# mmp/pbrt-v3

Measured on NVIDIA H100. Metric: Msamples/sec, higher is better.
Workload: dtype f32

## Files before the change

include/pb2.h:

```cpp
#ifndef PB2_H
#define PB2_H

#include <stddef.h>
#include <stdint.h>

#ifdef __cplusplus
extern "C" {
#endif

#define PB2_ABI_VERSION 10

typedef enum pb2_status {
    PB2_OK = 0,
    PB2_ERR_NO_DEVICE = 1,
    PB2_ERR_CUDA = 2,
    PB2_ERR_INVALID = 3,
    PB2_ERR_UNSUPPORTED = 4,
    PB2_ERR_NCCL = 5
} pb2_status;


typedef struct pb2_bvh_node {
    float bmin[3];
    float bmax[3];
    int32_t offset;
    uint16_t n_prims;
    uint8_t axis;
    uint8_t pad;
} pb2_bvh_node;

enum { PB2_PRIM_TRIANGLE = 0, PB2_PRIM_SPHERE = 1, PB2_PRIM_INSTANCE = 2 };
enum { PB2_MAT_NONE = 0, PB2_MAT_MATTE = 1, PB2_MAT_PLASTIC = 2, PB2_MAT_MIRROR = 3, PB2_MAT_GLASS = 4, PB2_MAT_SUBSTRATE = 5, PB2_MAT_METAL = 6,
       PB2_MAT_UBER = 7 };
enum { PB2_LIGHTDIST_UNIFORM = 0, PB2_LIGHTDIST_POWER = 1, PB2_LIGHTDIST_SPATIAL = 2 };
enum { PB2_FILTER_BOX = 0, PB2_FILTER_GAUSSIAN = 1, PB2_FILTER_MITCHELL = 2, PB2_FILTER_SINC = 3, PB2_FILTER_TRIANGLE = 4 };

typedef struct pb2_mesh {
    int32_t first_tri, n_tris;
    int32_t first_vertex, n_vertices;
    int32_t has_n, has_uv, has_s;
    int32_t reverse_orientation;
    int32_t transform_swaps_handedness;
    int32_t alpha_tex, shadow_alpha_tex;
    int32_t pad;
} pb2_mesh;

enum { PB2_WRAP_REPEAT = 0, PB2_WRAP_BLACK = 1, PB2_WRAP_CLAMP = 2 };
typedef struct pb2_texture {
    int32_t channels;
    int32_t width, height;
    int32_t wrap;
    int32_t do_trilinear;
    float max_anisotropy;
    float su, sv, du, dv;
    int32_t kind;
    int32_t pad;
    const float *texels;
    int32_t child[3];
    float value[3];
} pb2_texture;
enum { PB2_TEXKIND_IMAGE = 0, PB2_TEXKIND_CONSTANT = 1, PB2_TEXKIND_SCALE = 2, PB2_TEXKIND_MIX = 3, PB2_TEXKIND_CHECKERBOARD = 4,
       PB2_TEXKIND_UV = 5 };

enum { PB2_TEX_KD = 0, PB2_TEX_KS = 1, PB2_TEX_KR = 2, PB2_TEX_KT = 3, PB2_TEX_OPACITY = 4, PB2_TEX_SIGMA = 5, PB2_TEX_ROUGHNESS = 6,
       PB2_TEX_UROUGHNESS = 7, PB2_TEX_VROUGHNESS = 8, PB2_TEX_ETA = 9, PB2_TEX_METAL_ETA = 10, PB2_TEX_METAL_K = 11,
       PB2_TEX_BUMP = 12, PB2_TEX_SLOTS = 13 };

typedef struct pb2_sphere {
    float object_to_world[16];
    float world_to_object[16];
    float radius, z_min, z_max, theta_min, theta_max, phi_max;
    int32_t reverse_orientation;
    int32_t transform_swaps_handedness;
} pb2_sphere;

typedef struct pb2_material {
    int32_t type;
    float kd[3];
    float sigma;
    float ks[3];
    float roughness;
    int32_t remap_roughness;
    int32_t pad[2];
    float kr[3];
    float kt[3];
    float eta;
    float uroughness, vroughness;
    float opacity[3];
    float metal_eta[3];
    float metal_k[3];
    int32_t pad3[2];
    int32_t tex[16];
} pb2_material;

enum { PB2_LIGHT_AREA = 0, PB2_LIGHT_POINT = 1, PB2_LIGHT_SPOT = 2, PB2_LIGHT_DISTANT = 3, PB2_LIGHT_INFINITE = 4 };
typedef struct pb2_light {
    int32_t prim;
    float L[3];
    int32_t two_sided;
    float area;
    int32_t type;
    int32_t pad;
} pb2_light;

typedef struct pb2_delta_light {
    float p[3];
    float total_width_deg;
    float falloff_start_deg;
    float world_radius;
    float world_to_light[9];
    float pad;
    float light_to_world[9];
    int32_t env_tex;
    float pad2[2];
} pb2_delta_light;

typedef struct pb2_bvh {
    int64_t node_offset, n_nodes;
    int64_t prim_offset, n_prims;
} pb2_bvh;

typedef struct pb2_instance {
    float instance_to_world[16];
    float world_to_instance[16];
    int32_t bvh;
    int32_t lone_prim;
    int32_t pad[2];
} pb2_instance;

typedef struct pb2_scene_desc {
    int64_t n_vertices;
    const float *P;
    const float *N;
    const float *UV;
    const float *S;
    int64_t n_tris;
    const int32_t *tri_index;
    const int32_t *tri_mesh;
    int32_t n_meshes;
    const pb2_mesh *meshes;
    int32_t n_spheres;
    const pb2_sphere *spheres;

    int64_t n_prims;
    const uint8_t *prim_type;
    const int32_t *prim_index;
    const int32_t *prim_material;
    const int32_t *prim_light;

    int64_t n_nodes;
    const pb2_bvh_node *nodes;
    const int32_t *bvh_prims;

    int32_t n_materials;
    const pb2_material *materials;
    int32_t n_lights;
    const pb2_light *lights;

    int32_t light_strategy;
    int32_t spatial_max_voxels;

    int32_t n_instances;
    int32_t n_bvhs;
    const pb2_instance *instances;
    const pb2_bvh *bvhs;
    int64_t n_bvh_prims;
    const pb2_delta_light *delta_lights;
    int32_t n_textures;
    int32_t pad_textures;
    const pb2_texture *textures;
} pb2_scene_desc;

typedef struct pb2_camera {
    float camera_to_world[16];
    float world_to_camera[16];
    float screen_window[4];
    float fov;
    float lens_radius, focal_distance;
    float shutter_open, shutter_close;
    float raster_to_camera[16];
    float dx_camera[3], dy_camera[3];
} pb2_camera;

typedef struct pb2_film_desc {
    int32_t full_resolution[2];
    int32_t cropped_pixel_bounds[4];
    float filter_radius[2];
    float max_sample_luminance;
    float scale;
    int32_t filter_type;
    float filter_param[2];
    int32_t pad;
} pb2_film_desc;

typedef struct pb2_path_params {
    int32_t samples_per_pixel;
    int32_t sample_at_pixel_center;
    int32_t max_depth;
    float rr_threshold;
    int32_t pixel_bounds[4];
    int32_t tile_rank, tile_count;
    int32_t flags;
    int32_t sampler;
} pb2_path_params;

enum { PB2_SAMPLER_HALTON = 0, PB2_SAMPLER_SOBOL = 1 };

#define PB2_FLAG_COUNT_TRAVERSAL 1
#define PB2_FLAG_LINEAR_NODES 2
#define PB2_FLAG_WIDE4 4
#define PB2_FLAG_PLAIN_TRACE 8
#define PB2_FLAG_SMALL_STACK 16
#define PB2_FLAG_LD128 32
#define PB2_FLAG_LEAF_TMA 64
#define PB2_FLAG_POOL 128
#define PB2_FLAG_CHAIN 256

typedef struct pb2_ray {
    float o[3];
    float d[3];
    float t_max;
} pb2_ray;

typedef struct pb2_hit {
    int32_t prim;
    float t;
    float b[3];
    float p[3];
    float p_error[3];
    float n[3];
    float ns[3];
    float dpdu[3];
    float uv[2];
} pb2_hit;

typedef struct pb2_stats {
    uint64_t camera_rays;
    uint64_t regular_rays;
    uint64_t shadow_rays;
    uint64_t node_visits;
    uint64_t prim_tests;
    uint64_t kernel_launches;
    double render_ms;
    double h2d_ms, d2h_ms;
    double trace_ms;
} pb2_stats;

typedef struct pb2_scene pb2_scene;


int pb2_abi_version(void);
const char *pb2_last_error(void);

int pb2_init(int device_id);
int pb2_init_devices(int n_devices, const int *device_ids);
int pb2_device_count(void);
int pb2_shutdown(void);

#define PB2_DIST_ID_BYTES 128
int pb2_dist_unique_id(void *id);
int pb2_dist_init(int rank, int world, const void *id);
int pb2_dist_info(int *rank, int *world);
int pb2_dist_shutdown(void);

int pb2_work_items(const pb2_film_desc *film, const pb2_path_params *params, int64_t first, int64_t n, int32_t *out,
                   int64_t *n_items);

int pb2_host_alloc(size_t bytes, void **out);
int pb2_host_free(void *p);

int pb2_scene_create(const pb2_scene_desc *desc, pb2_scene **out);
int pb2_scene_destroy(pb2_scene *scene);
int pb2_shade_class(const pb2_scene_desc *desc, int32_t *out);

int pb2_intersect(pb2_scene *scene, const pb2_ray *rays, int64_t n, pb2_hit *hits);
int pb2_intersect_p(pb2_scene *scene, const pb2_ray *rays, int64_t n, uint8_t *occluded);

int pb2_render_path(pb2_scene *scene, const pb2_camera *camera, const pb2_film_desc *film,
                    const pb2_path_params *params, float *film_rgbw, pb2_stats *stats);

int pb2_render_path_device(pb2_scene *scene, const pb2_camera *camera, const pb2_film_desc *film,
                           const pb2_path_params *params, float *film_rgbw_device, int clear,
                           void *stream, pb2_stats *stats);

typedef struct pb2_wf_hit {
    int32_t found;
    int32_t leaf;
    int32_t prim;
    float t;
    float b[3];
    int32_t listed;
} pb2_wf_hit;
int pb2_trace_wavefront(pb2_scene *scene, const pb2_ray *rays, const uint8_t *any_hit, int64_t n, int32_t flags,
                        pb2_wf_hit *out);

int pb2_li_samples(pb2_scene *scene, const pb2_camera *camera, const pb2_film_desc *film,
                   const pb2_path_params *params, const int32_t *pixel_xy, const int64_t *sample_num,
                   int64_t n, float *out_rgb, float *out_pfilm);

int pb2_halton_samples(const pb2_film_desc *film, const pb2_path_params *params,
                       const int32_t *pixel_xy, const int64_t *sample_num, const int32_t *dim,
                       int64_t n, float *out);

int pb2_sobol_samples_host(const pb2_film_desc *film, const pb2_path_params *params, const int32_t *pixel_xy,
                           const int64_t *sample_num, const int32_t *dim, int64_t n, float *out, uint64_t *tables);

int pb2_light_distribution(pb2_scene *scene, const float *points_xyz, int64_t n, float *out);

int pb2_texture_pyramid(const pb2_texture *texture, int32_t level, int32_t *n_levels, int32_t *w, int32_t *h, float *out);

int pb2_texture_eval_host(const pb2_texture *textures, int32_t n_textures, int32_t id, int64_t n, const float *uv, const float *duv,
                          float *out);

int pb2_bsdf_eval_host(const pb2_material *material, int64_t n, const float *in, float *out);

int pb2_camera_differentials_host(const pb2_camera *camera, const pb2_film_desc *film, const pb2_path_params *params, int64_t n,
                                  const float *in, float *out);
int pb2_uv_differentials_host(int64_t n, const float *in, float *out);

int pb2_env_distribution(const pb2_texture *texture, int32_t *nu, int32_t *nv, float *out);

int pb2_texture_lookup(const pb2_texture *texture, int64_t n, const float *st, const float *dst, float *out);

typedef struct pb2_build_node {
    float bmin[3], bmax[3];
    int32_t child[2];
    int32_t split_axis;
    int32_t first_prim_offset;
    int32_t n_primitives;
} pb2_build_node;
int pb2_hlbvh_treelets(const float *prim_bounds, int64_t n, int32_t max_prims_in_node, pb2_build_node *pool,
                       int32_t *ordered_prims, int32_t *treelet_roots, int32_t *n_treelets, double *device_ms);

int pb2_hlbvh_build(const float *prim_bounds, int64_t n, int32_t max_prims_in_node, pb2_bvh_node *nodes, int64_t *n_nodes,
                    int32_t *ordered_prims, double *device_ms);

#ifdef __cplusplus
}
#endif
#endif
```

pbrt_v3_b200/csrc/pb2_cuda.cu:

```cuda
#include <cuda_runtime.h>
#include <cub/device/device_radix_sort.cuh>
#include <dlfcn.h>
#include <nccl.h>

#include <algorithm>
#include <mutex>
#include <chrono>
#include <cstddef>
#include <cstdio>
#include <cstdlib>
#include <cstring>
#include <string>
#include <thread>
#include <vector>

#include "device/pb2_path.cuh"
#include "device/pb2_wide4.cuh"
#include "host/core.h"
#include "pb2.h"

using namespace pb2;

static thread_local std::string g_lastError;
static int setError(int code, const std::string &msg) {
// ... 486 lines not shown
    int s = r >> 8, m = r & 255;
    int x = rp.sbx0 + tx * 16 + compact1by1((unsigned)m);
    int y = rp.sby0 + ty * 16 + compact1by1((unsigned)m >> 1);
    *px = x;
    *py = y;
    *sample = s;
    if (x >= rp.sbx1 || y >= rp.sby1) return false;
    return x >= rp.pbx0 && x < rp.pbx1 && y >= rp.pby0 && y < rp.pby1;
}

__device__ __noinline__ void addSampleFiltered(const DRenderParams &rp, float4 *film, V2 pFilm, V3 L) {
    float dx = pFilm.x - 0.5f, dy = pFilm.y - 0.5f;
    int p0x = (int)ceilf(dx - rp.filterRadiusX), p0y = (int)ceilf(dy - rp.filterRadiusY);
    int p1x = (int)floorf(dx + rp.filterRadiusX) + 1, p1y = (int)floorf(dy + rp.filterRadiusY) + 1;
    p0x = max(p0x, rp.cx0);
    p0y = max(p0y, rp.cy0);
    p1x = min(p1x, rp.cx1);
    p1y = min(p1y, rp.cy1);
    int width = rp.cx1 - rp.cx0;
    for (int yy = p0y; yy < p1y; ++yy) {
        float fy = fabsf(((float)yy - dy) * rp.invFilterRadiusY * 16.f);
        int ify = min((int)floorf(fy), 15);
        for (int xx = p0x; xx < p1x; ++xx) {
            float fx = fabsf(((float)xx - dx) * rp.invFilterRadiusX * 16.f);
            int ifx = min((int)floorf(fx), 15);
            float w = rp.filterTable[ify * 16 + ifx];
            float4 *px = film + ((size_t)(yy - rp.cy0) * width + (xx - rp.cx0));
            atomicAdd(px, make_float4(L.x * w, L.y * w, L.z * w, w));
        }
    }
}

__device__ __forceinline__ void addSample(const DRenderParams &rp, float4 *film, V2 pFilm, V3 L) {
    float y = luminance(L);
    if (y > rp.maxSampleLuminance) L = L * (rp.maxSampleLuminance / y);
    if (rp.filterTable) {
        addSampleFiltered(rp, film, pFilm, L);
        return;
    }
    float dx = pFilm.x - 0.5f, dy = pFilm.y - 0.5f;
    int p0x = (int)ceilf(dx - rp.filterRadiusX), p0y = (int)ceilf(dy - rp.filterRadiusY);
    int p1x = (int)floorf(dx + rp.filterRadiusX) + 1, p1y = (int)floorf(dy + rp.filterRadiusY) + 1;
    p0x = max(p0x, rp.cx0);
    p0y = max(p0y, rp.cy0);
    p1x = min(p1x, rp.cx1);
    p1y = min(p1y, rp.cy1);
    int width = rp.cx1 - rp.cx0;
    for (int yy = p0y; yy < p1y; ++yy)
        for (int xx = p0x; xx < p1x; ++xx) {
            float4 *px = film + ((size_t)(yy - rp.cy0) * width + (xx - rp.cx0));
            atomicAdd(px, make_float4(L.x, L.y, L.z, 1.f));
        }
}

#include "pb2_wavefront.cuh"

__global__ void k_li_samples(DScene sc, DRenderParams rp, const int32_t *pixelXY, const int64_t *sampleNum, int64_t n,
                             float *outRGB, float *outPFilm, int *deferred) {
    int64_t i = blockIdx.x * (int64_t)blockDim.x + threadIdx.x;
    if (i >= n) return;
    int px = pixelXY[2 * i], py = pixelXY[2 * i + 1];
    DSampler smp;
    smp.index = sampleIndex<true>(rp.halton, px, py, sampleNum[i]);
    smp.dim = 0;
    V2 pFilm;
    DRay ray = generateCameraRay<true>(rp.cam, rp.halton, smp, px, py, &pFilm);
    DLane ln;
    laneStartPath(ln, ray, smp);
    while (ln.state != LS_IDLE) {
        DHit hit;
        float tMax;
        bool found = traceLane(sc, ln, &tMax, &hit, nullptr);
        DTexCtx tc;
        tc.cam = &rp.cam;
        tc.pFilm = pFilm;
        tc.diffScale = rp.diffScale;
        laneAdvance<SHADE_FULL>(sc, rp.halton, rp.path, ln, found, hit, tMax, &tc);
        if (ln.state == LS_DEFER) {
            atomicAdd(deferred, 1);
            return;
        }
    }
    V3 L = guardRadiance(ln.L);
    outRGB[3 * i] = L.x;
    outRGB[3 * i + 1] = L.y;
    outRGB[3 * i + 2] = L.z;
    if (outPFilm) {
        outPFilm[2 * i] = pFilm.x;
        outPFilm[2 * i + 1] = pFilm.y;
    }
}

__global__ void k_wf_debug_fill(WfPool pool, const pb2_ray *rays, const uint8_t *anyHit, int n) {
    int i = blockIdx.x * blockDim.x + threadIdx.x;
    if (i == 0) {
        for (int q = 0; q < WQ_COUNT; ++q) pool.counts[q] = 0;
        pool.counts[WQ_TRACE0] = (unsigned)n;
    }
    if (i >= n) return;
    WfCtx &cx = pool.ctx[i];
    cx.ln.state = (anyHit && anyHit[i]) ? LS_SHADOW : LS_PATH;
    cx.ln.ray.o = mk3(rays[i].o[0], rays[i].o[1], rays[i].o[2]);
    cx.ln.ray.d = mk3(rays[i].d[0], rays[i].d[1], rays[i].d[2]);
    cx.ln.ray.tMax = rays[i].t_max;
    cx.hit = make_float4(__int_as_float(-1), 0.f, 0.f, 0.f);
    cx.tHit = 0.f;
    cx.found = -1;
    pool.queue[WQ_TRACE0][i] = i;
}
__global__ void k_wf_debug_read(DScene sc, WfPool pool, int n, pb2_wf_hit *out) {
    int i = blockIdx.x * blockDim.x + threadIdx.x;
    if (i >= n) return;
    const WfCtx &cx = pool.ctx[i];
    pb2_wf_hit h;
    h.found = cx.found;
    h.t = cx.tHit;
    h.leaf = __float_as_int(cx.hit.x);
    h.b[0] = cx.hit.y; h.b[1] = cx.hit.z; h.b[2] = cx.hit.w;
    h.prim = (cx.found > 0 && h.leaf >= 0) ? asInt(ldg4(&sc.leafPrims[3 * (size_t)h.leaf]).w) : -1;
    h.listed = 0;
    out[i] = h;
}
__global__ void k_wf_debug_lists(WfPool pool, pb2_wf_hit *out) {
    unsigned ns = pool.counts[WQ_SHADE], nl = pool.counts[WQ_LIGHT];
    for (unsigned i = blockIdx.x * blockDim.x + threadIdx.x; i < ns + nl; i += gridDim.x * blockDim.x) {
        int c = i < ns ? pool.queue[WQ_SHADE][i] : pool.queue[WQ_LIGHT][i - ns];
        atomicAdd(&out[c].listed, i < ns ? 1 : 2);
    }
}

__global__ void k_halton_samples(DHalton h, const int32_t *pixelXY, const int64_t *sampleNum, const int32_t *dim, int64_t n,
                                 float *out) {
    int64_t i = blockIdx.x * (int64_t)blockDim.x + threadIdx.x;
    if (i >= n) return;
    const int px = pixelXY[2 * i], py = pixelXY[2 * i + 1];
    int64_t index = sampleIndex<true>(h, px, py, sampleNum[i]);
    if (h.sobol && dim[i] < 2) out[i] = sobolPixelSample(h, index, dim[i], dim[i] == 0 ? px : py);
    else out[i] = sampleDimension<true>(h, index, dim[i]);
}

__global__ void k_halton_batch(DHalton h, const int32_t *pixelXY, const int64_t *sampleNum, const int32_t *dim0, int64_t n, float *out) {
    int64_t i = blockIdx.x * (int64_t)blockDim.x + threadIdx.x;
    if (i >= n) return;
    const int64_t index = sampleIndex<true>(h, pixelXY[2 * i], pixelXY[2 * i + 1], sampleNum[i]);
    float u[kSampleBatch];
    haltonSampleBatch<true>(h, index, dim0[i], kSampleBatch, u);
#pragma unroll
    for (int k = 0; k < kSampleBatch; ++k) out[kSampleBatch * i + k] = u[k];
}

__global__ void k_light_distribution(DScene sc, const float *points, int64_t n, float *out) {
    int64_t i = blockIdx.x * (int64_t)blockDim.x + threadIdx.x;
    if (i >= n) return;
    const float *rec = lightDistLookup(sc.lightDist, mk3(points[3 * i], points[3 * i + 1], points[3 * i + 2]));
    if (!rec) return;
    int stride = 2 * sc.nLights + 1;
    for (int k = 0; k < stride; ++k) out[i * stride + k] = rec[k];
}

static DHalton haltonTablesOnly() {
    DHalton h;
    memset(&h, 0, sizeof(h));
    h.primes = cur().primes;
    h.primeSums = cur().primeSums;
    h.perms = cur().perms;
    h.dimRecs = cur().dimRecs;
    h.dimTabs = cur().dimTabs;
    h.digitTab = cur().digitTab;
    return h;
}

static void launchLightDistBuild(const pb2_scene *scene, cudaStream_t stream) {
    k_lightdist_build<<<g_numSMs * 4, 128, 0, stream>>>(scene->d, haltonTablesOnly());
    k_lightdist_done<<<1, 32, 0, stream>>>(scene->d);
}
static int lightDistOverflowed(pb2_scene *scene, cudaStream_t stream, bool *overflowed) {
    *overflowed = false;
    if (!scene->lazyLightDist) return PB2_OK;
    CUDA_TRY(cudaMemcpyAsync(scene->ldHostCounters, scene->d.lightDist.counters, 4 * sizeof(int), cudaMemcpyDeviceToHost, stream));
    CUDA_TRY(cudaStreamSynchronize(stream));
    *overflowed = scene->ldHostCounters[2] != 0;
    return PB2_OK;
}
static int lightDistOverflowError() {
    return setError(PB2_ERR_UNSUPPORTED, "the on-demand pool of spatial light distributions is exhausted (very many lights x very many voxels touched): "
                                         "raise PB2_LIGHTDIST_POOL_MB or use lightsamplestrategy \"power\" / \"uniform\"");
}

static int requireDevice() {
    if (!g_initialised) return setError(PB2_ERR_NO_DEVICE, "pb2_init() has not succeeded: no CUDA device is bound (there is no CPU fallback)");
    return PB2_OK;
}

static bool computeFilterTable(const pb2_film_desc *f, float table[256]) {
    const float rx = f->filter_radius[0], ry = f->filter_radius[1];
    const float p0 = f->filter_param[0], p1 = f->filter_param[1];
    auto eval = [&](float x, float y) -> float {
        switch (f->filter_type) {
        case PB2_FILTER_GAUSSIAN: {
            const float alpha = p0, expX = std::exp(-alpha * rx * rx), expY = std::exp(-alpha * ry * ry);
            auto g = [&](float d, float expv) { return std::max((float)0, float(std::exp(-alpha * d * d) - expv)); };
            return g(x, expX) * g(y, expY);
        }
        case PB2_FILTER_MITCHELL: {
            const float B = p0, C = p1;
            auto m1 = [&](float v) {
                v = std::abs(2 * v);
                if (v > 1)
                    return ((-B - 6 * C) * v * v * v + (6 * B + 30 * C) * v * v + (-12 * B - 48 * C) * v + (8 * B + 24 * C)) * (1.f / 6.f);
                return ((12 - 9 * B - 6 * C) * v * v * v + (-18 + 12 * B + 6 * C) * v * v + (6 - 2 * B)) * (1.f / 6.f);
            };
            const float invRx = 1 / rx, invRy = 1 / ry;
            return m1(x * invRx) * m1(y * invRy);
        }
        case PB2_FILTER_SINC: {
            const float tau = p0, Pi = 3.14159265358979323846f;
            auto sinc = [&](float v) -> float {
                v = std::abs(v);
                if (v < 1e-5) return 1;
                return std::sin(Pi * v) / (Pi * v);
            };
            auto ws = [&](float v, float radius) -> float {
                v = std::abs(v);
                if (v > radius) return 0;
                float lanczos = sinc(v / tau);
                return sinc(v) * lanczos;
            };
            return ws(x, rx) * ws(y, ry);
        }
        case PB2_FILTER_TRIANGLE:
            return std::max((float)0, rx - std::abs(x)) * std::max((float)0, ry - std::abs(y));
        default:
            return 1.f;
        }
    };
    int offset = 0;
    for (int y = 0; y < 16; ++y)
        for (int x = 0; x < 16; ++x, ++offset) table[offset] = eval((x + 0.5f) * rx / 16, (y + 0.5f) * ry / 16);
    return f->filter_type != PB2_FILTER_BOX;
}

static DRenderParams makeRenderParams(const pb2_camera *cam, const pb2_film_desc *film, const pb2_path_params *pp) {
    DRenderParams rp;
    memset(&rp, 0, sizeof(rp));
    memcpy(rp.cam.rasterToCamera.m, cam->raster_to_camera, sizeof(float) * 16);
    memcpy(rp.cam.cameraToWorld.m, cam->camera_to_world, sizeof(float) * 16);
    rp.cam.lensRadius = cam->lens_radius;
    rp.cam.focalDistance = cam->focal_distance;
    rp.cam.dxCamera = mk3(cam->dx_camera[0], cam->dx_camera[1], cam->dx_camera[2]);
    rp.cam.dyCamera = mk3(cam->dy_camera[0], cam->dy_camera[1], cam->dy_camera[2]);
    rp.diffScale = 1 / std::sqrt((float)pp->samples_per_pixel);
    rp.halton = makeHalton(film, pp);
    rp.path.maxDepth = pp->max_depth;
    rp.path.rrThreshold = pp->rr_threshold;
    SampleBounds sb = filmSampleBounds(film);
    rp.sbx0 = sb.x0; rp.sby0 = sb.y0; rp.sbx1 = sb.x1; rp.sby1 = sb.y1;
    rp.pbx0 = pp->pixel_bounds[0]; rp.pby0 = pp->pixel_bounds[1]; rp.pbx1 = pp->pixel_bounds[2]; rp.pby1 = pp->pixel_bounds[3];
    rp.cx0 = film->cropped_pixel_bounds[0]; rp.cy0 = film->cropped_pixel_bounds[1];
    rp.cx1 = film->cropped_pixel_bounds[2]; rp.cy1 = film->cropped_pixel_bounds[3];
    rp.filterRadiusX = film->filter_radius[0];
    rp.filterRadiusY = film->filter_radius[1];
    rp.invFilterRadiusX = 1.f / film->filter_radius[0];
    rp.invFilterRadiusY = 1.f / film->filter_radius[1];
    rp.filterTable = nullptr;
    rp.maxSampleLuminance = film->max_sample_luminance;
    rp.nTilesX = (sb.x1 - sb.x0 + 15) / 16;
    rp.nTilesY = (sb.y1 - sb.y0 + 15) / 16;
    rp.tileCount = std::max(1, pp->tile_count);
    rp.tileRank = pp->tile_rank;
    long long nTiles = (long long)std::max(0, rp.nTilesX) * std::max(0, rp.nTilesY);
    rp.nOwnedTiles = nTiles > rp.tileRank ? (nTiles - rp.tileRank + rp.tileCount - 1) / rp.tileCount : 0;
    rp.spp = pp->samples_per_pixel;
    rp.nWorkItems = rp.nOwnedTiles * 256LL * rp.spp;
    return rp;
}

static int validateRenderArgs(const pb2_scene *scene, const pb2_camera *cam, const pb2_film_desc *film, const pb2_path_params *pp) {
    if (!scene || !cam || !film || !pp) return setError(PB2_ERR_INVALID, "null argument");
    if (pp->samples_per_pixel <= 0 || pp->max_depth < 0) return setError(PB2_ERR_INVALID, "bad samples_per_pixel / max_depth");
    if (5 + 8 * ((long long)pp->max_depth + 1) > kMaxHaltonDims)
        return setError(PB2_ERR_UNSUPPORTED, "maxdepth above 123: HaltonSampler can only sample 1000 dimensions");
    if (pp->tile_count < 0 || pp->tile_rank < 0 || (pp->tile_count > 0 && pp->tile_rank >= pp->tile_count))
        return setError(PB2_ERR_INVALID, "bad tile_rank / tile_count");
    if (pp->sampler != PB2_SAMPLER_HALTON && pp->sampler != PB2_SAMPLER_SOBOL) return setError(PB2_ERR_INVALID, "unknown sampler");
    if (pp->sampler == PB2_SAMPLER_SOBOL && (pp->samples_per_pixel & (pp->samples_per_pixel - 1)))
        return setError(PB2_ERR_INVALID, "SobolSampler: samples_per_pixel must be the power of two its constructor rounds up to (sobol.h:52)");
    if (film->cropped_pixel_bounds[2] < film->cropped_pixel_bounds[0] || film->cropped_pixel_bounds[3] < film->cropped_pixel_bounds[1])
        return setError(PB2_ERR_INVALID, "bad cropped pixel bounds");
    if (!(film->filter_radius[0] > 0) || !(film->filter_radius[1] > 0)) return setError(PB2_ERR_INVALID, "bad filter radius");
    if (film->filter_type < PB2_FILTER_BOX || film->filter_type > PB2_FILTER_TRIANGLE) return setError(PB2_ERR_INVALID, "unknown filter type");
    return PB2_OK;
}

enum { kMaxPipes = 4 };
typedef void (*TraceKernel)(DScene, WfPool, int, WfChain);
typedef void (*AdvanceKernel)(const DScene *, const DRenderParams *, WfPool, int, int, int, float4 *, unsigned long long *);

struct TraceLaunch {
    TraceKernel fn = nullptr;
    int block = 128;
    size_t smem = 0;
    int grid = 0;
    bool chain = false;
    const char *name = "";
};

enum TraceKernelForm { TK_COUNT, TK_PLAIN, TK_POOL, TK_WIDE2, TK_WIDE4, TK_LINEAR };
struct TraceKernelEntry {
    TraceKernelForm form;
    int features;
    TraceKernel fn;
    const char *name;
    size_t smem;
};
template <int WIDTH, int T>
static TraceKernelEntry wideTrace() {
    const char *name = WIDTH == 4              ? "k_wf_trace_w<4>"
                       : (T & TRACE_ALPHA) ? "k_wf_trace_w<2,alpha>"
                       : (T & TRACE_CHAIN) ? "k_wf_trace_w<2,chain>"
                                           : "k_wf_trace_w<2>";
    return {WIDTH == 4 ? TK_WIDE4 : TK_WIDE2, T, k_wf_trace_w<WIDTH, T>, name, 0};
}
template <int T>
static TraceKernelEntry linearTrace() { return {TK_LINEAR, T, k_wf_trace<T>, "k_wf_trace", 0}; }

struct TraceKey {
    TraceKernelForm form;
    int features;
};
static TraceKey chooseTraceKernel(const pb2_scene *scene, int flags, bool render) {
    const bool instanced = scene->d.instances != nullptr;
    const bool records = scene->d.wide4 != nullptr && !(flags & PB2_FLAG_LINEAR_NODES);
    const bool linearFits = !instanced || scene->bvhDepth + 3 + scene->instDepth <= 64;
    int sceneBits = scene->d.spheres ? TRACE_SPHERES : 0;
    if (instanced) sceneBits |= TRACE_SPHERES | TRACE_INST;
    if (flags & PB2_FLAG_COUNT_TRAVERSAL) return {TK_COUNT, 0};
    if ((flags & PB2_FLAG_PLAIN_TRACE) || (!records && !linearFits)) return {TK_PLAIN, 0};
    if (scene->d.hasAlpha) return records ? TraceKey{TK_WIDE2, sceneBits | TRACE_ALPHA} : TraceKey{TK_PLAIN, 0};
    if (!records) return {TK_LINEAR, sceneBits | (sceneBits || scene->bvhDepth > 32 ? TRACE_DEEP : 0)};
    if ((flags & PB2_FLAG_POOL) && !sceneBits) return {TK_POOL, 0};
    const bool ld128 = (flags & PB2_FLAG_LD128) != 0;
    int features = sceneBits | (ld128 ? TRACE_LD128 : 0) | ((flags & PB2_FLAG_SMALL_STACK) ? TRACE_SMALL_STACK : 0);
    if (flags & PB2_FLAG_WIDE4) return {TK_WIDE4, features};
    if (!ld128 && (flags & PB2_FLAG_LEAF_TMA) && !sceneBits) features = TRACE_LEAF_TMA;
    if (!ld128 && render && (flags & PB2_FLAG_CHAIN) && !(flags & (PB2_FLAG_SMALL_STACK | PB2_FLAG_LEAF_TMA))) features |= TRACE_CHAIN;
    return {TK_WIDE2, features};
}

static int selectTraceKernel(pb2_scene *scene, int flags, TraceLaunch *out, bool render = false, const char *steps = "") {
    static const TraceKernelEntry kernels[] = {
        {TK_COUNT, 0, k_wf_trace_plain<true>, "k_wf_trace_plain<count>", 0},
        {TK_PLAIN, 0, k_wf_trace_plain<false>, "k_wf_trace_plain", 0},
        {TK_POOL, 0, k_wf_trace_pool, "k_wf_trace_pool", 4 * sizeof(PoolWarp)},
        wideTrace<2, 0>(), wideTrace<2, TRACE_SMALL_STACK>(),
        wideTrace<2, TRACE_LD128>(), wideTrace<2, TRACE_LD128 | TRACE_SMALL_STACK>(),
        wideTrace<2, TRACE_SPHERES>(), wideTrace<2, TRACE_SPHERES | TRACE_SMALL_STACK>(),
        wideTrace<2, TRACE_SPHERES | TRACE_LD128>(), wideTrace<2, TRACE_SPHERES | TRACE_LD128 | TRACE_SMALL_STACK>(),
        wideTrace<2, TRACE_SPHERES | TRACE_INST>(), wideTrace<2, TRACE_SPHERES | TRACE_INST | TRACE_SMALL_STACK>(),
        wideTrace<2, TRACE_SPHERES | TRACE_INST | TRACE_LD128>(), wideTrace<2, TRACE_SPHERES | TRACE_INST | TRACE_LD128 | TRACE_SMALL_STACK>(),
        wideTrace<2, TRACE_LEAF_TMA>(),
        wideTrace<2, TRACE_CHAIN>(), wideTrace<2, TRACE_SPHERES | TRACE_CHAIN>(), wideTrace<2, TRACE_SPHERES | TRACE_INST | TRACE_CHAIN>(),
        wideTrace<2, TRACE_ALPHA>(), wideTrace<2, TRACE_SPHERES | TRACE_ALPHA>(), wideTrace<2, TRACE_SPHERES | TRACE_INST | TRACE_ALPHA>(),
        wideTrace<4, 0>(), wideTrace<4, TRACE_SMALL_STACK>(),
        wideTrace<4, TRACE_LD128>(), wideTrace<4, TRACE_LD128 | TRACE_SMALL_STACK>(),
        wideTrace<4, TRACE_SPHERES>(), wideTrace<4, TRACE_SPHERES | TRACE_SMALL_STACK>(),
        wideTrace<4, TRACE_SPHERES | TRACE_LD128>(), wideTrace<4, TRACE_SPHERES | TRACE_LD128 | TRACE_SMALL_STACK>(),
        wideTrace<4, TRACE_SPHERES | TRACE_INST>(), wideTrace<4, TRACE_SPHERES | TRACE_INST | TRACE_SMALL_STACK>(),
        wideTrace<4, TRACE_SPHERES | TRACE_INST | TRACE_LD128>(), wideTrace<4, TRACE_SPHERES | TRACE_INST | TRACE_LD128 | TRACE_SMALL_STACK>(),
        linearTrace<0>(), linearTrace<TRACE_DEEP>(),
        linearTrace<TRACE_SPHERES | TRACE_DEEP>(), linearTrace<TRACE_SPHERES | TRACE_INST | TRACE_DEEP>(),
    };
    const TraceKey want = chooseTraceKernel(scene, flags, render);
    const TraceKernelEntry *k = nullptr;
    for (const TraceKernelEntry &e : kernels)
        if (e.form == want.form && e.features == want.features) k = &e;
    if (!k)
        return setError(PB2_ERR_CUDA, "no trace kernel of form " + std::to_string(want.form) + " is compiled for the trace features " +
                                          std::to_string(want.features));
    TraceLaunch t;
    t.fn = k->fn;
    t.smem = k->smem;
    t.chain = (k->features & TRACE_CHAIN) != 0;
    t.name = k->name;
    if (k->form == TK_POOL && !scene->wfSpill)
        CUDA_TRY(cudaMalloc((void **)&scene->wfSpill, (size_t)kMaxPipes * g_numSMs * 8 * 4 * PL_R * PL_SPILL * sizeof(int2)));
    if (t.smem) CUDA_TRY(cudaFuncSetAttribute(t.fn, cudaFuncAttributeMaxDynamicSharedMemorySize, (int)t.smem));
    int blocksPerSM = 1;
    CUDA_TRY(cudaOccupancyMaxActiveBlocksPerMultiprocessor(&blocksPerSM, t.fn, t.block, t.smem));
    blocksPerSM = std::max(1, std::min(blocksPerSM, 8));
    cudaFuncAttributes fa;
    CUDA_TRY(cudaFuncGetAttributes(&fa, t.fn));
    size_t need = (size_t)blocksPerSM * (fa.sharedSizeBytes + t.smem + 1024);
    int pct = (int)std::min<size_t>(100, (need * 100 + 233471) / 233472);
    CUDA_TRY(cudaFuncSetAttribute(t.fn, cudaFuncAttributePreferredSharedMemoryCarveout, pct));
    static const int verbose = envInt("PB2_VERBOSE", 0);
    if (verbose)
        fprintf(stderr, "pb2: trace kernel %s: %d regs, %zu B smem, %d blocks/SM, carve-out %d %%, BVH depth %d%s\n", t.name, fa.numRegs,
                fa.sharedSizeBytes + t.smem, blocksPerSM, pct, scene->bvhDepth, steps);
    t.grid = g_numSMs * blocksPerSM;
    *out = t;
    return PB2_OK;
}

static int ensurePool(pb2_scene *scene, int capacity) {
    if (scene->wfCapacity < capacity) {
        if (scene->wfCtx) cudaFree(scene->wfCtx);
        if (scene->wfQueues) cudaFree(scene->wfQueues);
        scene->wfCtx = nullptr;
        scene->wfQueues = nullptr;
        scene->wfCapacity = 0;
        CUDA_TRY(cudaMalloc(&scene->wfCtx, (size_t)capacity * sizeof(WfCtx)));
        CUDA_TRY(cudaMalloc((void **)&scene->wfQueues, (size_t)capacity * WQ_COUNT * sizeof(int)));
        scene->wfCapacity = capacity;
    }
    if (!scene->wfCounts) CUDA_TRY(cudaMalloc((void **)&scene->wfCounts, kMaxPipes * WQ_COUNT * sizeof(unsigned)));
    if (!scene->wfHostCounts) CUDA_TRY(cudaMallocHost((void **)&scene->wfHostCounts, (kMaxPipes * WQ_COUNT + 2) * sizeof(unsigned long long)));
    return PB2_OK;
}

static WfPool poolOf(const pb2_scene *scene, int capacity, int pipe = 0, int nPipes = 1) {
    WfPool pool;
    const int cap = capacity / nPipes;
    pool.capacity = cap;
    pool.ctx = (WfCtx *)scene->wfCtx + (size_t)pipe * cap;
    for (int q = 0; q < WQ_COUNT; ++q) pool.queue[q] = scene->wfQueues + ((size_t)pipe * WQ_COUNT + q) * cap;
    pool.counts = scene->wfCounts + (size_t)pipe * WQ_COUNT;
    pool.ctr = scene->counters;
    pool.spill = scene->wfSpill ? scene->wfSpill + (size_t)pipe * g_numSMs * 8 * 4 * PL_R * PL_SPILL : nullptr;
    return pool;
}

constexpr int kShadeLambertAreaMinBlocks = 4;

typedef void (*GenKernel)(const DRenderParams *, WfPool, int, int);
typedef void (*FinishKernel)(const DScene *, const DRenderParams *, WfPool, int, unsigned, float4 *);

template <typename K>
struct StepKernel {
    int features;
    K fn;
};
template <bool SHADE, int MINB, int F>
static StepKernel<AdvanceKernel> advanceStep() { return {F, k_wf_advance<SHADE, MINB, F>}; }

template <typename K, size_t N>
static const StepKernel<K> &stepKernel(const StepKernel<K> (&table)[N], int frame) {
    int reads = 0;
    for (const StepKernel<K> &k : table) reads |= k.features;
    const StepKernel<K> *best = nullptr;
    for (const StepKernel<K> &k : table)
        if (!(frame & reads & ~k.features) && (!best || __builtin_popcount(k.features) < __builtin_popcount(best->features))) best = &k;
    return *best;
}

static int frameShadeFeatures(const pb2_scene *scene, const DRenderParams &rp) {
    int f = scene->shadeFeatures;
    if (scene->d.spheres) f |= SHADE_SPHERES;
    if (scene->lazyLightDist) f |= SHADE_LAZY;
    if (scene->d.nTextures > 0) f |= SHADE_TEXTURES;
    if (rp.halton.sobol) f |= SHADE_SOBOL;
    return f;
}

static int renderWavefront(pb2_scene *scene, const DRenderParams &rp, float4 *film, cudaStream_t stream, int flags,
                           bool timeTrace, unsigned long long *launches, double *traceMs) {
    const bool lazyLights = scene->lazyLightDist;
    static const int maxCapacity = envInt("PB2_POOL", 1 << 22);
    long long want = std::min<long long>(maxCapacity, std::max<long long>(rp.nWorkItems, 1024));
    int capacity = (int)((want + 255) / 256 * 256);
    int rc = ensurePool(scene, capacity);
    if (rc) return rc;
    static const StepKernel<GenKernel> genSteps[] = {{0, k_wf_gen<0>}, {SHADE_SOBOL, k_wf_gen<SHADE_SOBOL>}};
    static const StepKernel<AdvanceKernel> lightSteps[] = {
        advanceStep<false, 7, SHADE_LAMBERT_AREA>(),
        advanceStep<false, 7, SHADE_GENERAL>(),
        advanceStep<false, 7, SHADE_GENERAL | SHADE_SPHERES>(),
    };
    static const StepKernel<AdvanceKernel> shadeSteps[] = {
        advanceStep<true, kShadeLambertAreaMinBlocks, SHADE_LAMBERT_AREA>(),
        advanceStep<true, 4, SHADE_GENERAL>(),
        advanceStep<true, 4, SHADE_GENERAL | SHADE_SPHERES>(),
        advanceStep<true, 4, SHADE_GENERAL | SHADE_SPECULAR>(),
        advanceStep<true, 4, SHADE_GENERAL | SHADE_SPHERES | SHADE_SPECULAR>(),
        advanceStep<true, 4, SHADE_GENERAL | SHADE_LAZY>(),
        advanceStep<true, 4, SHADE_GENERAL | SHADE_SPHERES | SHADE_LAZY>(),
        advanceStep<true, 4, SHADE_GENERAL | SHADE_SPECULAR | SHADE_LAZY>(),
        advanceStep<true, 4, SHADE_GENERAL | SHADE_SPHERES | SHADE_SPECULAR | SHADE_LAZY>(),
        advanceStep<true, 3, SHADE_FULL>(),
    };
    static const StepKernel<FinishKernel> finishSteps[] = {
        {SHADE_LAMBERT_AREA, k_wf_finish<SHADE_LAMBERT_AREA>},
        {SHADE_GENERAL, k_wf_finish<SHADE_GENERAL>},
        {SHADE_GENERAL | SHADE_SPHERES, k_wf_finish<SHADE_GENERAL | SHADE_SPHERES>},
        {SHADE_GENERAL | SHADE_SPECULAR, k_wf_finish<SHADE_GENERAL | SHADE_SPECULAR>},
        {SHADE_GENERAL | SHADE_SPHERES | SHADE_SPECULAR, k_wf_finish<SHADE_GENERAL | SHADE_SPHERES | SHADE_SPECULAR>},
    };
    const int features = frameShadeFeatures(scene, rp);
    const StepKernel<GenKernel> &gen = stepKernel(genSteps, features);
    const StepKernel<AdvanceKernel> &advLight = stepKernel(lightSteps, features), &advShade = stepKernel(shadeSteps, features);
    const StepKernel<FinishKernel> &finish = stepKernel(finishSteps, features);
    char steps[96];
    snprintf(steps, sizeof(steps), "; shade features %d: gen %d, light %d, shade %d, tail %d", features, gen.features,
             advLight.features, advShade.features, finish.features);
    TraceLaunch trace;
    if ((rc = selectTraceKernel(scene, flags, &trace, true, steps))) return rc;
    if (!scene->paramBuf) CUDA_TRY(cudaMalloc(&scene->paramBuf, sizeof(DScene) + sizeof(DRenderParams)));
    const DScene *dSc = reinterpret_cast<const DScene *>(scene->paramBuf);
    const DRenderParams *dRp = reinterpret_cast<const DRenderParams *>((char *)scene->paramBuf + sizeof(DScene));
    CUDA_TRY(cudaMemcpyAsync((void *)dSc, &scene->d, sizeof(DScene), cudaMemcpyHostToDevice, stream));
    CUDA_TRY(cudaMemcpyAsync((void *)dRp, &rp, sizeof(DRenderParams), cudaMemcpyHostToDevice, stream));
    WfChain chain;
    memset(&chain, 0, sizeof(chain));
    if (trace.chain) {
        chain.sc = dSc;
        chain.rp = dRp;
        chain.film = film;
    }
    static const int finishPerSM = envInt("PB2_FINISH", 256);
    const bool textured = (features & (SHADE_TEXTURES | SHADE_SOBOL)) != 0;
    const unsigned finishThreshold = ((flags & PB2_FLAG_COUNT_TRAVERSAL) || lazyLights || textured) ? 0u : (unsigned)(g_numSMs * std::max(0, finishPerSM));
    const int finishBlocks = std::max(1, (int)((finishThreshold + 127) / 128));
    static const int syncEvery = std::max(1, envInt("PB2_SYNC_EVERY", 8));
    static const int pipesEnv = envInt("PB2_PIPES", 0);
    const int pipesWanted = std::min((int)kMaxPipes, pipesEnv > 0 ? pipesEnv : 2);
    const int nPipes = (lazyLights || capacity < 65536) ? 1 : pipesWanted;
    cudaStream_t streams[kMaxPipes] = {stream, stream, stream, stream};
    if (nPipes > 1) {
        if (!scene->forkEvent) CUDA_TRY(cudaEventCreateWithFlags(&scene->forkEvent, cudaEventDisableTiming));
        CUDA_TRY(cudaEventRecord(scene->forkEvent, stream));
        for (int p = 1; p < nPipes; ++p) {
            if (!scene->pipeStreams[p]) CUDA_TRY(cudaStreamCreateWithFlags(&scene->pipeStreams[p], cudaStreamNonBlocking));
            if (!scene->joinEvents[p]) CUDA_TRY(cudaEventCreateWithFlags(&scene->joinEvents[p], cudaEventDisableTiming));
            streams[p] = scene->pipeStreams[p];
            CUDA_TRY(cudaStreamWaitEvent(streams[p], scene->forkEvent, 0));
        }
    }
    WfPool pools[kMaxPipes];
    for (int p = 0; p < nPipes; ++p) pools[p] = poolOf(scene, capacity / nPipes * nPipes, p, nPipes);
    const int capP = pools[0].capacity;
    const int blocks128 = std::min((capP + 127) / 128, g_numSMs * 32);
    for (int p = 0; p < nPipes; ++p) k_wf_init<<<(capP + 255) / 256, 256, 0, streams[p]>>>(pools[p]);
    unsigned long long nLaunch = nPipes;
    size_t nEvents = 0;
    int cur = 0;
    volatile unsigned *hc = scene->wfHostCounts;
    unsigned long long *hWork = reinterpret_cast<unsigned long long *>(scene->wfHostCounts + kMaxPipes * WQ_COUNT);
    for (long long round = 0;; ++round) {
        int next = 1 - cur;
        for (int p = 0; p < nPipes; ++p) {
            const WfPool &pool = pools[p];
            cudaStream_t st = streams[p];
            gen.fn<<<blocks128, 128, 0, st>>>(dRp, pool, WQ_FREE0 + cur, WQ_TRACE0 + cur);
            if (timeTrace) {
                if (scene->traceEvents.size() < nEvents + 2) {
                    cudaEvent_t e0, e1;
                    CUDA_TRY(cudaEventCreate(&e0));
                    CUDA_TRY(cudaEventCreate(&e1));
                    scene->traceEvents.push_back(e0);
                    scene->traceEvents.push_back(e1);
                }
                CUDA_TRY(cudaEventRecord(scene->traceEvents[nEvents], st));
            }
            chain.freeQ = WQ_FREE0 + next;
            trace.fn<<<trace.grid, trace.block, trace.smem, st>>>(scene->d, pool, WQ_TRACE0 + cur, chain);
            if (timeTrace) {
                CUDA_TRY(cudaEventRecord(scene->traceEvents[nEvents + 1], st));
                nEvents += 2;
            }
            if (!trace.chain) advLight.fn<<<blocks128, 128, 0, st>>>(dSc, dRp, pool, WQ_LIGHT, WQ_TRACE0 + next, WQ_FREE0 + next, film, scene->counters);
            else --nLaunch;
            advShade.fn<<<blocks128, 128, 0, st>>>(dSc, dRp, pool, WQ_SHADE, WQ_TRACE0 + next, WQ_FREE0 + next, film, scene->counters);
            if (lazyLights) {
                launchLightDistBuild(scene, st);
                advShade.fn<<<blocks128, 128, 0, st>>>(dSc, dRp, pool, WQ_RETRY, WQ_TRACE0 + next, WQ_FREE0 + next, film, scene->counters);
                nLaunch += 3;
            }
            if (finishThreshold) finish.fn<<<finishBlocks, 128, 0, st>>>(dSc, dRp, pool, WQ_TRACE0 + next, finishThreshold, film);
            k_wf_reset<<<1, 32, 0, st>>>(pool, WQ_FREE0 + cur, WQ_TRACE0 + cur, WQ_TRACE0 + next, finishThreshold);
            nLaunch += finishThreshold ? 6 : 5;
        }
        cur = next;
        if ((round + 1) % syncEvery != 0) continue;
        for (int p = 0; p < nPipes; ++p)
            CUDA_TRY(cudaMemcpyAsync((void *)(scene->wfHostCounts + p * WQ_COUNT), pools[p].counts, WQ_COUNT * sizeof(unsigned), cudaMemcpyDeviceToHost, streams[p]));
        for (int p = 1; p < nPipes; ++p) CUDA_TRY(cudaStreamSynchronize(streams[p]));
        CUDA_TRY(cudaMemcpyAsync(hWork, &scene->counters[CTR_WORK], sizeof(unsigned long long), cudaMemcpyDeviceToHost, stream));
        CUDA_TRY(cudaStreamSynchronize(stream));
        bool overflowed = false;
        if ((rc = lightDistOverflowed(scene, stream, &overflowed))) return rc;
        if (overflowed) return lightDistOverflowError();
        const bool workLeft = (long long)*hWork < rp.nWorkItems;
        bool done = true;
        for (int p = 0; p < nPipes; ++p) {
            const unsigned traceNext = hc[p * WQ_COUNT + WQ_TRACE0 + cur], freeNext = hc[p * WQ_COUNT + WQ_FREE0 + cur];
            if (!(traceNext == 0 && !(workLeft && freeNext > 0))) done = false;
        }
        if (done) break;
        if (round > 100000000LL) return setError(PB2_ERR_CUDA, "wavefront did not terminate");
    }
    if (nPipes > 1) {
        for (int p = 1; p < nPipes; ++p) {
            CUDA_TRY(cudaEventRecord(scene->joinEvents[p], streams[p]));
            CUDA_TRY(cudaStreamWaitEvent(stream, scene->joinEvents[p], 0));
        }
    }
    CUDA_TRY(cudaGetLastError());
    *launches = nLaunch;
    *traceMs = 0;
    for (size_t e = 0; e + 1 < nEvents; e += 2) {
        float ms = 0;
        CUDA_TRY(cudaEventElapsedTime(&ms, scene->traceEvents[e], scene->traceEvents[e + 1]));
        *traceMs += ms;
    }
    return PB2_OK;
}

extern "C" {

int pb2_abi_version(void) { return PB2_ABI_VERSION; }
const char *pb2_last_error(void) { return g_lastError.c_str(); }

static void freeDeviceTables() {
    for (DeviceState &d : g_devs) {
        cudaSetDevice(d.id);
        cudaFree(d.primes);
        cudaFree(d.primeSums);
        cudaFree(d.perms);
        cudaFree(d.dimRecs);
        cudaFree(d.dimTabs);
        cudaFree(d.digitTab);
        cudaFree(d.sobol);
        cudaFree(d.sobolVdc);
    }
    g_devs.clear();
    g_initialised = false;
}

int pb2_init_devices(int n, const int *device_ids) {
    int count = 0;
    cudaError_t e = cudaGetDeviceCount(&count);
    if (e != cudaSuccess || count == 0) {
        cudaGetLastError();
        return setError(PB2_ERR_NO_DEVICE, std::string("no CUDA device available (") +
                                               (e != cudaSuccess ? cudaGetErrorString(e) : "device count is 0") +
                                               "); the path-tracing hot path has no CPU fallback");
    }
    std::vector<int> ids;
    if (n <= 0) for (int i = 0; i < count; ++i) ids.push_back(i);
    else {
        if (!device_ids) return setError(PB2_ERR_INVALID, "null device list");
        ids.assign(device_ids, device_ids + n);
    }
    for (size_t i = 0; i < ids.size(); ++i) {
        if (ids[i] < 0 || ids[i] >= count) return setError(PB2_ERR_INVALID, "device id out of range");
        for (size_t j = 0; j < i; ++j)
            if (ids[j] == ids[i]) return setError(PB2_ERR_INVALID, "device listed twice");
    }
    if (g_initialised && g_devs.size() == ids.size()) {
        bool same = true;
        for (size_t i = 0; i < ids.size(); ++i) same &= g_devs[i].id == ids[i];
        if (same) return PB2_OK;
    }
    if (g_dist.comm) return setError(PB2_ERR_INVALID, "pb2_init: shut the communicator down (pb2_dist_shutdown) before rebinding devices");
    freeDeviceTables();
    buildHaltonHostTables();
    t_dev = 0;
    for (int id : ids) {
        CUDA_TRY(cudaSetDevice(id));
        cudaDeviceProp prop;
        CUDA_TRY(cudaGetDeviceProperties(&prop, id));
        if (prop.major != 9 || prop.minor != 0) {
            freeDeviceTables();
            return setError(PB2_ERR_NO_DEVICE, std::string("device \"") + prop.name + "\" is not sm_90 (Hopper); this library is built for sm_90a only");
        }
        g_devs.emplace_back();
        DeviceState &d = g_devs.back();
        d.id = id;
        d.numSMs = prop.multiProcessorCount;
        CUDA_TRY(cudaMalloc((void **)&d.primes, g_halton.hPrimes.size() * sizeof(int32_t)));
        CUDA_TRY(cudaMalloc((void **)&d.primeSums, g_halton.hPrimeSums.size() * sizeof(int32_t)));
        CUDA_TRY(cudaMalloc((void **)&d.perms, g_halton.hPerms.size() * sizeof(uint16_t)));
        CUDA_TRY(cudaMalloc((void **)&d.dimRecs, g_halton.hDimRecs.size() * sizeof(ulonglong2)));
        CUDA_TRY(cudaMemcpy(d.dimRecs, g_halton.hDimRecs.data(), g_halton.hDimRecs.size() * sizeof(ulonglong2), cudaMemcpyHostToDevice));
        CUDA_TRY(cudaMemcpy(d.primes, g_halton.hPrimes.data(), g_halton.hPrimes.size() * sizeof(int32_t), cudaMemcpyHostToDevice));
        CUDA_TRY(cudaMemcpy(d.primeSums, g_halton.hPrimeSums.data(), g_halton.hPrimeSums.size() * sizeof(int32_t), cudaMemcpyHostToDevice));
        CUDA_TRY(cudaMemcpy(d.perms, g_halton.hPerms.data(), g_halton.hPerms.size() * sizeof(uint16_t), cudaMemcpyHostToDevice));
        CUDA_TRY(cudaMalloc((void **)&d.dimTabs, g_halton.hDimTabs.size() * sizeof(HaltonDimTab)));
        CUDA_TRY(cudaMalloc((void **)&d.digitTab, g_halton.hDigitTab.size() * sizeof(uint16_t)));
        CUDA_TRY(cudaMemcpy(d.dimTabs, g_halton.hDimTabs.data(), g_halton.hDimTabs.size() * sizeof(HaltonDimTab), cudaMemcpyHostToDevice));
        CUDA_TRY(cudaMemcpy(d.digitTab, g_halton.hDigitTab.data(), g_halton.hDigitTab.size() * sizeof(uint16_t), cudaMemcpyHostToDevice));
    }
    CUDA_TRY(cudaSetDevice(g_devs[0].id));
    for (size_t i = 1; i < g_devs.size(); ++i) {
        int can = 0;
        if (cudaDeviceCanAccessPeer(&can, g_devs[0].id, g_devs[i].id) == cudaSuccess && can) {
            cudaError_t pe = cudaDeviceEnablePeerAccess(g_devs[i].id, 0);
            g_devs[i].peerOfPrimary = pe == cudaSuccess || pe == cudaErrorPeerAccessAlreadyEnabled;
        }
        cudaGetLastError();
    }
    g_initialised = true;
    return PB2_OK;
}

int pb2_init(int device_id) { return pb2_init_devices(1, &device_id); }

int pb2_device_count(void) { return g_initialised ? (int)g_devs.size() : 0; }

int pb2_shutdown(void) {
    if (!g_initialised) return PB2_OK;
    pb2_dist_shutdown();
    freeDeviceTables();
    return PB2_OK;
}

int pb2_debug_radical_inverse_tables(const uint32_t *index, const int32_t *dim, int64_t n, float *out_loop, float *out_tab) {
    if (!index || !dim || !out_loop || !out_tab) return setError(PB2_ERR_INVALID, "null argument");
    buildHaltonHostTables();
    for (int64_t i = 0; i < n; ++i) {
        if (dim[i] < 2 || dim[i] >= kMaxHaltonDims) return setError(PB2_ERR_INVALID, "dimension out of range");
        const uint32_t base = (uint32_t)g_halton.hPrimes[dim[i]];
        const uint16_t *perm = g_halton.hPerms.data() + g_halton.hPrimeSums[dim[i]];
        const uint64_t magic = g_halton.hDimRecs[dim[i]].x;
        out_loop[i] = scrambledRadicalInverse32(base, magic, index[i], perm);
        out_tab[i] = scrambledRadicalInverseTab(g_halton.hDimTabs[dim[i]], g_halton.hDigitTab.data(), base, magic, index[i], perm);
    }
    return PB2_OK;
}

int pb2_debug_halton_batch(const pb2_film_desc *film, const pb2_path_params *pp, const uint32_t *index, const int32_t *dim0, int64_t n,
                           float *out_batch, float *out_tab) {
    if (!film || !pp || !index || !dim0 || !out_batch || !out_tab) return setError(PB2_ERR_INVALID, "null argument");
    buildHaltonHostTables();
    DHalton h = makeHalton(film, pp);
    h.perms = g_halton.hPerms.data();
    h.primes = g_halton.hPrimes.data();
    h.primeSums = g_halton.hPrimeSums.data();
    h.dimRecs = g_halton.hDimRecs.data();
    h.dimTabs = g_halton.hDimTabs.data();
    h.digitTab = g_halton.hDigitTab.data();
    for (int64_t i = 0; i < n; ++i) {
        if (dim0[i] < 2 || dim0[i] + kSampleBatch > kMaxHaltonDims) return setError(PB2_ERR_INVALID, "dimension out of range");
        haltonSampleBatch(h, (int64_t)index[i], dim0[i], kSampleBatch, out_batch + kSampleBatch * i);
        for (int k = 0; k < kSampleBatch; ++k) {
            const int d = dim0[i] + k;
            const uint32_t base = (uint32_t)g_halton.hPrimes[d];
            const uint16_t *perm = g_halton.hPerms.data() + g_halton.hPrimeSums[d];
            out_tab[kSampleBatch * i + k] = scrambledRadicalInverseTab(g_halton.hDimTabs[d], g_halton.hDigitTab.data(), base,
                                                                       g_halton.hDimRecs[d].x, index[i], perm);
        }
    }
    return PB2_OK;
}

int pb2_debug_halton_batch_device(const pb2_film_desc *film, const pb2_path_params *pp, const int32_t *pixel_xy,
                                  const int64_t *sample_num, const int32_t *dim0, int64_t n, float *out) {
    int rc = requireDevice();
    if (rc) return rc;
    if (!film || !pp || (n > 0 && (!pixel_xy || !sample_num || !dim0 || !out))) return setError(PB2_ERR_INVALID, "null argument");
    if (n <= 0) return PB2_OK;
    for (int64_t i = 0; i < n; ++i)
        if (dim0[i] < 0 || dim0[i] + kSampleBatch > kMaxHaltonDims) return setError(PB2_ERR_INVALID, "dimension out of range");
    DHalton h = makeHalton(film, pp);
    if (pp->sampler == PB2_SAMPLER_SOBOL && (rc = attachSobol(&h, film))) return rc;
    int32_t *dXY = nullptr, *dDim = nullptr;
    int64_t *dS = nullptr;
    float *dOut = nullptr;
    cudaError_t e = cudaMalloc((void **)&dXY, n * 2 * sizeof(int32_t));
    if (e == cudaSuccess) e = cudaMalloc((void **)&dS, n * sizeof(int64_t));
    if (e == cudaSuccess) e = cudaMalloc((void **)&dDim, n * sizeof(int32_t));
    if (e == cudaSuccess) e = cudaMalloc((void **)&dOut, n * kSampleBatch * sizeof(float));
    if (e == cudaSuccess) e = cudaMemcpy(dXY, pixel_xy, n * 2 * sizeof(int32_t), cudaMemcpyHostToDevice);
    if (e == cudaSuccess) e = cudaMemcpy(dS, sample_num, n * sizeof(int64_t), cudaMemcpyHostToDevice);
    if (e == cudaSuccess) e = cudaMemcpy(dDim, dim0, n * sizeof(int32_t), cudaMemcpyHostToDevice);
    if (e == cudaSuccess) {
        k_halton_batch<<<(unsigned)((n + 127) / 128), 128>>>(h, dXY, dS, dDim, n, dOut);
        e = cudaGetLastError();
    }
    if (e == cudaSuccess) e = cudaMemcpy(out, dOut, n * kSampleBatch * sizeof(float), cudaMemcpyDeviceToHost);
    cudaFree(dXY);
    cudaFree(dS);
    cudaFree(dDim);
    cudaFree(dOut);
    if (e != cudaSuccess) return setError(PB2_ERR_CUDA, std::string("pb2_debug_halton_batch_device: ") + cudaGetErrorString(e));
    return PB2_OK;
}

int pb2_work_items(const pb2_film_desc *film, const pb2_path_params *pp, int64_t first, int64_t n, int32_t *out, int64_t *n_items) {
    if (!film || !pp) return setError(PB2_ERR_INVALID, "null argument");
    if (pp->samples_per_pixel <= 0 || pp->tile_count < 0 || pp->tile_rank < 0 || (pp->tile_count > 0 && pp->tile_rank >= pp->tile_count))
        return setError(PB2_ERR_INVALID, "bad samples_per_pixel / tile_rank / tile_count");
    pb2_camera cam;
    memset(&cam, 0, sizeof(cam));
    const DRenderParams rp = makeRenderParams(&cam, film, pp);
    if (n_items) *n_items = rp.nWorkItems;
    for (int64_t i = 0; i < n && out; ++i) {
        int px = -1, py = -1, sample = -1;
        const bool inside = first + i >= 0 && first + i < rp.nWorkItems && decodeWork(rp, first + i, &px, &py, &sample);
        out[3 * i] = inside ? px : -1;
        out[3 * i + 1] = inside ? py : -1;
        out[3 * i + 2] = inside ? sample : -1;
    }
    return PB2_OK;
}

int pb2_dist_unique_id(void *id128) {
    if (!id128) return setError(PB2_ERR_INVALID, "null argument");
    int rc = loadNccl();
    if (rc) return rc;
    static_assert(sizeof(ncclUniqueId) == PB2_DIST_ID_BYTES, "ncclUniqueId is 128 bytes");
    ncclUniqueId id;
    NCCL_TRY(g_nccl.GetUniqueId(&id));
    memcpy(id128, &id, sizeof(id));
    return PB2_OK;
}

int pb2_dist_init(int rank, int world, const void *id128) {
    int rc = requireDevice();
    if (rc) return rc;
    if (world < 1 || rank < 0 || rank >= world || (world > 1 && !id128)) return setError(PB2_ERR_INVALID, "bad rank / world / id");
    if (g_dist.comm) return setError(PB2_ERR_INVALID, "pb2_dist_init: a communicator already exists (call pb2_dist_shutdown first)");
    g_dist.rank = rank;
    g_dist.world = world;
    if (world == 1) return PB2_OK;
    if ((rc = loadNccl())) return rc;
    ncclUniqueId id;
    memcpy(&id, id128, sizeof(id));
    if (g_devs.size() != 1) return setError(PB2_ERR_INVALID, "pb2_dist_init: one device per process (pb2_init), not a local device group");
// ... 1843 lines not shown
```

Measured before the change: 222.6.

## Reserve SM room for a shading block beside persistent trace blocks across pipes

When two pipelines run and shading is simple Lambert/area, the trace kernel's blocks per SM are reduced so that one block of the gen/light/shade kernels still fits in registers, threads and shared memory. The intent is to let the other pipe's list kernels run concurrently with the persistent trace grid instead of waiting for it. It also sets matching shared-memory carveouts on the list kernels so the SM partition does not need reconfiguring between them. The cost is fewer resident trace blocks, and the benefit depends on overlap really happening across the streams.

```diff
diff --git a/include/pb2.h b/include/pb2.h
--- a/include/pb2.h
+++ b/include/pb2.h
@@ -294,6 +294,8 @@
 int pb2_trace_wavefront(pb2_scene *scene, const pb2_ray *rays, const uint8_t *any_hit, int64_t n, int32_t flags,
                         pb2_wf_hit *out);
 
+int pb2_trace_blocks_with_reserve(int32_t trace_regs, int32_t trace_smem, int32_t list_regs, int32_t list_smem, int32_t max_blocks);
+
 int pb2_li_samples(pb2_scene *scene, const pb2_camera *camera, const pb2_film_desc *film,
                    const pb2_path_params *params, const int32_t *pixel_xy, const int64_t *sample_num,
                    int64_t n, float *out_rgb, float *out_pfilm);
diff --git a/pbrt_v3_b200/csrc/pb2_cuda.cu b/pbrt_v3_b200/csrc/pb2_cuda.cu
--- a/pbrt_v3_b200/csrc/pb2_cuda.cu
+++ b/pbrt_v3_b200/csrc/pb2_cuda.cu
@@ -812,6 +812,8 @@
     size_t smem = 0;
     int grid = 0;
     bool chain = false;
+    int carveout = 0;
+    bool reserved = false;
     const char *name = "";
 };
 
@@ -857,7 +859,31 @@
     return {TK_WIDE2, features};
 }
 
-static int selectTraceKernel(pb2_scene *scene, int flags, TraceLaunch *out, bool render = false, const char *steps = "") {
+constexpr int kSmRegs = 65536, kSmThreads = 2048, kSmBlocks = 32, kRegUnit = 256;
+constexpr int kSmSmem = 233472, kBlockSmemReserved = 1024;
+
+static int blockRegs(int regsPerThread, int threads) {
+    return (threads + 31) / 32 * ((regsPerThread * 32 + kRegUnit - 1) / kRegUnit * kRegUnit);
+}
+
+static int carveoutPercent(size_t bytes) { return (int)std::min<size_t>(100, (bytes * 100 + kSmSmem - 1) / kSmSmem); }
+
+extern "C" int pb2_trace_blocks_with_reserve(int32_t traceRegs, int32_t traceSmem, int32_t listRegs, int32_t listSmem, int32_t maxBlocks) {
+    const int list = blockRegs(listRegs, 128), trace = blockRegs(traceRegs, 128);
+    int n = std::min(maxBlocks, kSmBlocks - 1);
+    while (n > 0 && (n * trace + list > kSmRegs || (n + 1) * 128 > kSmThreads ||
+                     n * (traceSmem + kBlockSmemReserved) + listSmem + kBlockSmemReserved > kSmSmem))
+        --n;
+    return std::max(n, 0);
+}
+
+struct ListReserve {
+    int regs = 0;
+    int smem = 0;
+};
+
+static int selectTraceKernel(pb2_scene *scene, int flags, TraceLaunch *out, bool render = false, const char *steps = "",
+                             const ListReserve *reserve = nullptr) {
     static const TraceKernelEntry kernels[] = {
         {TK_COUNT, 0, k_wf_trace_plain<true>, "k_wf_trace_plain<count>", 0},
         {TK_PLAIN, 0, k_wf_trace_plain<false>, "k_wf_trace_plain", 0},
@@ -896,17 +922,28 @@
         CUDA_TRY(cudaMalloc((void **)&scene->wfSpill, (size_t)kMaxPipes * g_numSMs * 8 * 4 * PL_R * PL_SPILL * sizeof(int2)));
     if (t.smem) CUDA_TRY(cudaFuncSetAttribute(t.fn, cudaFuncAttributeMaxDynamicSharedMemorySize, (int)t.smem));
     int blocksPerSM = 1;
+    CUDA_TRY(cudaFuncSetAttribute(t.fn, cudaFuncAttributePreferredSharedMemoryCarveout, (int)cudaSharedmemCarveoutMaxShared));
     CUDA_TRY(cudaOccupancyMaxActiveBlocksPerMultiprocessor(&blocksPerSM, t.fn, t.block, t.smem));
-    blocksPerSM = std::max(1, std::min(blocksPerSM, 8));
+    const int maxBlocks = std::max(1, std::min(blocksPerSM, 8));
     cudaFuncAttributes fa;
     CUDA_TRY(cudaFuncGetAttributes(&fa, t.fn));
-    size_t need = (size_t)blocksPerSM * (fa.sharedSizeBytes + t.smem + 1024);
-    int pct = (int)std::min<size_t>(100, (need * 100 + 233471) / 233472);
-    CUDA_TRY(cudaFuncSetAttribute(t.fn, cudaFuncAttributePreferredSharedMemoryCarveout, pct));
+    const int traceSmem = (int)(fa.sharedSizeBytes + t.smem);
+    if (maxBlocks < 8) reserve = nullptr;
+    t.reserved = reserve != nullptr;
+    blocksPerSM = reserve ? std::max(1, pb2_trace_blocks_with_reserve(fa.numRegs, traceSmem, reserve->regs, reserve->smem, maxBlocks)) : maxBlocks;
+    const int fixedBlocks = envInt("PB2_TRACE_BLOCKS", 0);
+    if (fixedBlocks > 0) blocksPerSM = std::min(fixedBlocks, maxBlocks);
+    size_t need = (size_t)blocksPerSM * (traceSmem + kBlockSmemReserved);
+    if (reserve) need += reserve->smem + kBlockSmemReserved;
+    t.carveout = carveoutPercent(need);
+    CUDA_TRY(cudaFuncSetAttribute(t.fn, cudaFuncAttributePreferredSharedMemoryCarveout, t.carveout));
     static const int verbose = envInt("PB2_VERBOSE", 0);
-    if (verbose)
-        fprintf(stderr, "pb2: trace kernel %s: %d regs, %zu B smem, %d blocks/SM, carve-out %d %%, BVH depth %d%s\n", t.name, fa.numRegs,
-                fa.sharedSizeBytes + t.smem, blocksPerSM, pct, scene->bvhDepth, steps);
+    if (verbose) {
+        char room[96] = "";
+        if (reserve) snprintf(room, sizeof(room), " (reserve: one list block of %d regs, %d B smem)", reserve->regs, reserve->smem);
+        fprintf(stderr, "pb2: trace kernel %s: %d regs, %d B smem, %d blocks/SM%s, carve-out %d %%, BVH depth %d%s\n", t.name, fa.numRegs,
+                traceSmem, blocksPerSM, room, t.carveout, scene->bvhDepth, steps);
+    }
     t.grid = g_numSMs * blocksPerSM;
     *out = t;
     return PB2_OK;
@@ -1012,8 +1049,24 @@
     char steps[96];
     snprintf(steps, sizeof(steps), "; shade features %d: gen %d, light %d, shade %d, tail %d", features, gen.features,
              advLight.features, advShade.features, finish.features);
+    static const int pipesEnv = envInt("PB2_PIPES", 0);
+    const int pipesWanted = std::min((int)kMaxPipes, pipesEnv > 0 ? pipesEnv : 2);
+    const int nPipes = (lazyLights || capacity < 65536) ? 1 : pipesWanted;
+    const bool share = nPipes > 1 && advShade.features == SHADE_LAMBERT_AREA;
+    ListReserve reserve;
+    if (share) {
+        for (const void *fn : {(const void *)gen.fn, (const void *)advLight.fn, (const void *)advShade.fn}) {
+            cudaFuncAttributes fa;
+            CUDA_TRY(cudaFuncGetAttributes(&fa, fn));
+            reserve.regs = std::max(reserve.regs, fa.numRegs);
+            reserve.smem = std::max(reserve.smem, (int)fa.sharedSizeBytes);
+        }
+    }
     TraceLaunch trace;
-    if ((rc = selectTraceKernel(scene, flags, &trace, true, steps))) return rc;
+    if ((rc = selectTraceKernel(scene, flags, &trace, true, steps, share ? &reserve : nullptr))) return rc;
+    const int listCarveout = trace.reserved ? trace.carveout : (int)cudaSharedmemCarveoutDefault;
+    for (const void *fn : {(const void *)gen.fn, (const void *)advLight.fn, (const void *)advShade.fn, (const void *)finish.fn, (const void *)k_wf_reset})
+        CUDA_TRY(cudaFuncSetAttribute(fn, cudaFuncAttributePreferredSharedMemoryCarveout, listCarveout));
     if (!scene->paramBuf) CUDA_TRY(cudaMalloc(&scene->paramBuf, sizeof(DScene) + sizeof(DRenderParams)));
     const DScene *dSc = reinterpret_cast<const DScene *>(scene->paramBuf);
     const DRenderParams *dRp = reinterpret_cast<const DRenderParams *>((char *)scene->paramBuf + sizeof(DScene));
@@ -1031,9 +1084,6 @@
     const unsigned finishThreshold = ((flags & PB2_FLAG_COUNT_TRAVERSAL) || lazyLights || textured) ? 0u : (unsigned)(g_numSMs * std::max(0, finishPerSM));
     const int finishBlocks = std::max(1, (int)((finishThreshold + 127) / 128));
     static const int syncEvery = std::max(1, envInt("PB2_SYNC_EVERY", 8));
-    static const int pipesEnv = envInt("PB2_PIPES", 0);
-    const int pipesWanted = std::min((int)kMaxPipes, pipesEnv > 0 ? pipesEnv : 2);
-    const int nPipes = (lazyLights || capacity < 65536) ? 1 : pipesWanted;
     cudaStream_t streams[kMaxPipes] = {stream, stream, stream, stream};
     if (nPipes > 1) {
         if (!scene->forkEvent) CUDA_TRY(cudaEventCreateWithFlags(&scene->forkEvent, cudaEventDisableTiming));
```

After: 234.4 (median of 6 runs). +5.3%, better.
